# wg-perception/PartsBasedDetector

Measured on AMD Instinct MI355X. Metric: detect() frames/sec, 640x480, 26-part person model, higher is better.
Workload: dtype f32

## Files before the change

partsbaseddetector_amd/csrc/k_conv.hip:

```cpp
#include <algorithm>
#include <vector>
#include <cstring>
#include "pbd_internal.hpp"
#include <type_traits>
#include "k_conv_mfma16.hpp"

#ifdef PBD_PROBES
bool conv_variants_debug_read(unsigned long long* out);
void conv_debug_read(unsigned long long* out) {
  if (!conv_variants_debug_read(out)) hipMemcpyFromSymbol(out, HIP_SYMBOL(pbd_conv_dbg), sizeof(unsigned long long) * 8);
}
#else
void conv_debug_read(unsigned long long* out) { for (int i = 0; i < 8; ++i) out[i] = 0; }
#endif

#define CSTR 33
#define NFG 8

template <int KH, int KW>
__device__ __forceinline__ void stage_feature_tile(float* __restrict__ ft, const float* __restrict__ F, int y0, int x0,
                                                   int H, int W, int tid) {
  constexpr int TW = CT + KW - 1, TH = CT + KH - 1, N = TH * TW * 8, NB = (N + 255) / 256;
  float4 r[NB];
#pragma unroll
  for (int j = 0; j < NB; ++j) {
    const int i = min(tid + j * 256, N - 1);
    const int cell = i >> 3, q = i & 7;
    const int ty = cell / TW, tx = cell - ty * TW;
    const int y = min(max(y0 + ty - KH / 2, 0), H - 1), x = min(max(x0 + tx - KW / 2, 0), W - 1);
    r[j] = *(const float4*)(F + ((size_t)y * W + x) * PBD_FLEN + q * 4);
  }
#pragma unroll
  for (int j = 0; j < NB; ++j) {
    const int i = tid + j * 256;
    if (i < N) {
      const int cell = i >> 3, q = i & 7;
      const int ty = cell / TW, tx = cell - ty * TW;
      const int y = y0 + ty - KH / 2, x = x0 + tx - KW / 2;
      float4 v = r[j];
      if (!(y >= 0 && y < H && x >= 0 && x < W)) v = make_float4(0.f, 0.f, 0.f, q == 7 ? 1.f : 0.f);
      float* d = ft + cell * CSTR + q * 4;
      d[0] = v.x; d[1] = v.y; d[2] = v.z; d[3] = v.w;
    }
  }
}

template <int KH, int KW>
__global__ __launch_bounds__(256) void k_conv_exact(const ConvTile* __restrict__ tiles,
                                                    const LevelDev* __restrict__ levels,
                                                    const float* __restrict__ feat, const float* __restrict__ wT,
                                                    float* __restrict__ resp, int nf, int nfpad, int groups_per_wg) {
  extern __shared__ __attribute__((aligned(16))) char smem[];
  typedef float T;
  T* ft = (T*)smem;
  const ConvTile t = tiles[blockIdx.x];
  const LevelDev lv = levels[t.level];
  const int H = lv.ch, W = lv.cw;
  const int TW = CT + KW - 1;
  const int tid = threadIdx.x;
  const T* F = feat + lv.cell_off * PBD_FLEN;
  stage_feature_tile<KH, KW>(ft, F, t.y0, t.x0, H, W, tid);
  __syncthreads();
  const int ly = tid >> 4, lx = tid & 15;
  const int oy = t.y0 + ly, ox = t.x0 + lx;
  const bool valid = (oy < H && ox < W);
  const T* fbase = ft + (ly * TW + lx) * CSTR;
  T* R = resp + lv.cell_off * nf;
  const int g0 = blockIdx.y * groups_per_wg;
  for (int g = g0; g < g0 + groups_per_wg; ++g) {
    const int n0 = g * NFG;
    if (n0 >= nf) break;
    T tot[NFG];
#pragma unroll
    for (int n = 0; n < NFG; ++n) tot[n] = (T)0;
    for (int c = 0; c < PBD_FLEN; ++c) {
      T acc[NFG];
#pragma unroll
      for (int n = 0; n < NFG; ++n) acc[n] = (T)0;
#pragma unroll
      for (int i = 0; i < KH; ++i) {
#pragma unroll
        for (int j = 0; j < KW; ++j) {
          const T f = fbase[(i * TW + j) * CSTR + c];
          const T* w = wT + ((size_t)(i * KW + j) * PBD_FLEN + c) * nfpad + n0;
#pragma unroll
          for (int n = 0; n < NFG; ++n) acc[n] += w[n] * f;
        }
      }
#pragma unroll
      for (int n = 0; n < NFG; ++n) tot[n] += acc[n];
    }
    if (valid) {
#pragma unroll
      for (int n = 0; n < NFG; ++n)
        if (n0 + n < nf) R[(size_t)(n0 + n) * H * W + (size_t)oy * W + ox] = tot[n];
    }
  }
}

#define CHALF 16
#define CSTRH 17
template <int KH, int KW, int GPW>
__global__ __launch_bounds__(256) void k_conv_exact_f64(const ConvTile* __restrict__ tiles,
                                                        const LevelDev* __restrict__ levels,
                                                        const double* __restrict__ feat, const double* __restrict__ wT,
                                                        double* __restrict__ resp, int nf, int nfpad) {
  extern __shared__ __attribute__((aligned(16))) char smem[];
  double* ft = (double*)smem;
  const ConvTile t = tiles[blockIdx.x];
  const LevelDev lv = levels[t.level];
  const int H = lv.ch, W = lv.cw;
  constexpr int TW = CT + KW - 1;
  const int tid = threadIdx.x;
  const double* F = feat + lv.cell_off * PBD_FLEN;
  const int ly = tid >> 4, lx = tid & 15;
  const int oy = t.y0 + ly, ox = t.x0 + lx;
  const bool valid = (oy < H && ox < W);
  const double* fbase = ft + (ly * TW + lx) * CSTRH;
  double* R = resp + lv.cell_off * nf;
  const int g0 = blockIdx.y * GPW;
  double tot[GPW][NFG];
#pragma unroll
  for (int g = 0; g < GPW; ++g)
#pragma unroll
    for (int n = 0; n < NFG; ++n) tot[g][n] = 0.0;
  for (int half = 0; half < PBD_FLEN / CHALF; ++half) {
    if (half) __syncthreads();
    stage_tile<double, CHALF, CSTRH, 7>(ft, F, t.y0, t.x0, H, W, KH, KW, half * CHALF, half == PBD_FLEN / CHALF - 1, tid);
    __syncthreads();
#pragma unroll
    for (int g = 0; g < GPW; ++g) {
      const int n0 = (g0 + g) * NFG;
      if (n0 >= nf) break;
      for (int cc = 0; cc < CHALF; ++cc) {
        const int c = half * CHALF + cc;
        double acc[NFG];
#pragma unroll
        for (int n = 0; n < NFG; ++n) acc[n] = 0.0;
#pragma unroll
        for (int i = 0; i < KH; ++i) {
#pragma unroll
          for (int j = 0; j < KW; ++j) {
            const double f = fbase[(i * TW + j) * CSTRH + cc];
            const double* w = wT + ((size_t)(i * KW + j) * PBD_FLEN + c) * nfpad + n0;
#pragma unroll
            for (int n = 0; n < NFG; ++n) acc[n] += w[n] * f;
          }
        }
#pragma unroll
        for (int n = 0; n < NFG; ++n) tot[g][n] += acc[n];
      }
    }
  }
  if (valid) {
#pragma unroll
    for (int g = 0; g < GPW; ++g) {
      const int n0 = (g0 + g) * NFG;
#pragma unroll
      for (int n = 0; n < NFG; ++n)
        if (n0 + n < nf) R[(size_t)(n0 + n) * H * W + (size_t)oy * W + ox] = tot[g][n];
    }
  }
}

template <typename T, bool MIX = false>
__global__ __launch_bounds__(256) void k_conv_exact_generic(const ConvTile* __restrict__ tiles,
                                                            const LevelDev* __restrict__ levels,
                                                            const T* __restrict__ feat,
                                                            const T* __restrict__ wT, T* __restrict__ resp,
                                                            int nf, int nfpad, int KH, int KW) {
  extern __shared__ __attribute__((aligned(16))) char smem[];
  T* ft = (T*)smem;
  const ConvTile t = tiles[blockIdx.x];
  const LevelDev lv = levels[t.level];
  const int H = lv.ch, W = lv.cw;
  const int TW = CT + KW - 1, TH = CT + KH - 1;
  const int tid = threadIdx.x;
  const T* F = feat + lv.cell_off * PBD_FLEN;
  for (int i = tid; i < TH * TW * PBD_FLEN; i += 256) {
    const int cell = i >> 5, c = i & 31;
    const int ty = cell / TW, tx = cell - ty * TW;
    const int y = t.y0 + ty - KH / 2, x = t.x0 + tx - KW / 2;
    const bool inside = (y >= 0 && y < H && x >= 0 && x < W);
    const T v = F[((size_t)min(max(y, 0), H - 1) * W + min(max(x, 0), W - 1)) * PBD_FLEN + c];
    ft[cell * CSTR + c] = inside ? v : (T)(c == PBD_FLEN - 1 ? 1 : 0);
  }
  __syncthreads();
  const int ly = tid >> 4, lx = tid & 15;
  const int oy = t.y0 + ly, ox = t.x0 + lx;
  const bool valid = (oy < H && ox < W);
  const T* fbase = ft + (ly * TW + lx) * CSTR;
  T* R = resp + lv.cell_off * nf;
  int nfw = nf;
  if constexpr (MIX) { R += (size_t)(t.pad & 0xFFFF) * H * W; nfw = t.pad >> 16; }
  for (int n = blockIdx.y; n < nfw; n += gridDim.y) {
    T tot = (T)0;
    for (int c = 0; c < PBD_FLEN; ++c) {
      T acc = (T)0;
      for (int i = 0; i < KH; ++i)
        for (int j = 0; j < KW; ++j)
          acc += wT[((size_t)(i * KW + j) * PBD_FLEN + c) * nfpad + n] * fbase[(i * TW + j) * CSTR + c];
      tot += acc;
    }
    if (valid) R[(size_t)n * H * W + (size_t)oy * W + ox] = tot;
  }
}

template <typename T>
static void launch_conv_exact_t(const ConvTile* tiles, int ntiles, const LevelDev* levels, const T* feat,
                                const T* wT, T* resp, int nf, int nfpad, int kh, int kw, hipStream_t s, int nf_stride) {
  const size_t lds = sizeof(T) * (CT + kh - 1) * (CT + kw - 1) * CSTR;
  if (nf_stride > 0) {
    static LdsOptIn optinm;
    optinm.ensure((const void*)k_conv_exact_generic<T, true>, lds);
    dim3 grid(ntiles, nf < 16 ? nf : 16);
    hipLaunchKernelGGL((k_conv_exact_generic<T, true>), grid, dim3(256), lds, s, tiles, levels, feat, wT, resp, nf_stride, nfpad, kh, kw);
    return;
  }
  if (kh == 5 && kw == 5) {
    const int groups = (nf + NFG - 1) / NFG;
    constexpr int GPW = 4;
    dim3 grid(ntiles, (groups + GPW - 1) / GPW);
    static LdsOptIn optin;
    if constexpr (sizeof(T) == 8) {
      const size_t ldsh = sizeof(double) * (CT + 4) * (CT + 4) * CSTRH;
      optin.ensure((const void*)k_conv_exact_f64<5, 5, GPW>, ldsh);
      hipLaunchKernelGGL((k_conv_exact_f64<5, 5, GPW>), grid, dim3(256), ldsh, s, tiles, levels, feat, wT, resp, nf, nfpad);
    } else {
      optin.ensure((const void*)k_conv_exact<5, 5>, lds);
      hipLaunchKernelGGL((k_conv_exact<5, 5>), grid, dim3(256), lds, s, tiles, levels, feat, wT, resp, nf, nfpad, GPW);
    }
  } else {
    static LdsOptIn opting;
    opting.ensure((const void*)k_conv_exact_generic<T>, lds);
    dim3 grid(ntiles, nf < 16 ? nf : 16);
    hipLaunchKernelGGL(k_conv_exact_generic<T>, grid, dim3(256), lds, s, tiles, levels, feat, wT, resp, nf, nfpad, kh, kw);
  }
}

void launch_conv_exact(const ConvTile* tiles, int ntiles, const LevelDev* levels, const void* feat, const void* wT,
                       void* resp, int ts, int nf, int nfpad, int kh, int kw, hipStream_t s, int nf_stride) {
  if (ntiles <= 0) return;
  if (ts == 8) launch_conv_exact_t<double>(tiles, ntiles, levels, (const double*)feat, (const double*)wT, (double*)resp, nf, nfpad, kh, kw, s, nf_stride);
  else launch_conv_exact_t<float>(tiles, ntiles, levels, (const float*)feat, (const float*)wT, (float*)resp, nf, nfpad, kh, kw, s, nf_stride);
}

void launch_conv_mfma_f64(const ConvTile* tiles, int ntiles, const LevelDev* levels, const double* feat,
                          const double* w4u, double* resp, int nf, int nfpad, int kh, int kw, hipStream_t s, int nf_stride) {
  if (ntiles <= 0) return;
  if (nf_stride > 0)
    launch_conv_mfma16_t<double, 4, 2, 1, true, 0, 0, true>(tiles, ntiles, levels, feat, w4u, resp, nf, nfpad, s, kh, kw, nf_stride);
  else if (kh != 5 || kw != 5)
    launch_conv_mfma16_t<double, 4, 2, 1, true, 0, 0>(tiles, ntiles, levels, feat, w4u, resp, nf, nfpad, s, kh, kw);
  else
    launch_conv_mfma16_t<double, 4, 2, 1, true>(tiles, ntiles, levels, feat, w4u, resp, nf, nfpad, s);
}

void launch_conv_mfma16_f32(const ConvTile* tiles, int ntiles, const LevelDev* levels, const float* feat,
                            const float* w4u, float* resp, int nf, int nfpad, int kh, int kw, hipStream_t s, int nf_stride) {
  if (ntiles <= 0) return;
  if (nf_stride > 0)
    launch_conv_mfma16_t<float, 2, 3, 2, true, 0, 0, true>(tiles, ntiles, levels, feat, w4u, resp, nf, nfpad, s, kh, kw, nf_stride);
  else if (kh != 5 || kw != 5)
    launch_conv_mfma16_t<float, 2, 3, 2, true, 0, 0>(tiles, ntiles, levels, feat, w4u, resp, nf, nfpad, s, kh, kw);
  else
    launch_conv_mfma16_t<float, 2, 3, 2, true>(tiles, ntiles, levels, feat, w4u, resp, nf, nfpad, s);
}
```

Baseline: 2440.

## Rework f32 5x5 conv inner loop with packed float2 FMAs and prefetching

The f32 5x5 exact conv kernel now computes 16 filters per group using packed float2 vector math instead of 8 scalar filters. Weights for the next tap are loaded one step ahead through constant-address-space pointers, and feature values for the next channel are prefetched from LDS. Scheduling barriers pin the loads between FMA groups. The aim is to raise FMA throughput via packed ops and hide weight/LDS load latency. In exchange it uses more registers, which may lower occupancy, and the grid is rebalanced to 2 groups per workgroup.

New measurement: 2445, median of 2. Within noise of the previous version (+0.2%).

```diff
diff --git a/partsbaseddetector_amd/csrc/k_conv.hip b/partsbaseddetector_amd/csrc/k_conv.hip
--- a/partsbaseddetector_amd/csrc/k_conv.hip
+++ b/partsbaseddetector_amd/csrc/k_conv.hip
@@ -16,6 +16,9 @@
 
 #define CSTR 33
 #define NFG 8
+#define NFGP 16
+typedef float float2v __attribute__((ext_vector_type(2)));
+typedef const __attribute__((address_space(4))) float2v* wpair_ptr;
 
 template <int KH, int KW>
 __device__ __forceinline__ void stage_feature_tile(float* __restrict__ ft, const float* __restrict__ F, int y0, int x0,
@@ -66,34 +69,59 @@
   const bool valid = (oy < H && ox < W);
   const T* fbase = ft + (ly * TW + lx) * CSTR;
   T* R = resp + lv.cell_off * nf;
+  const size_t wtap = (size_t)PBD_FLEN * nfpad;
   const int g0 = blockIdx.y * groups_per_wg;
   for (int g = g0; g < g0 + groups_per_wg; ++g) {
-    const int n0 = g * NFG;
+    const int n0 = g * NFGP;
     if (n0 >= nf) break;
-    T tot[NFG];
-#pragma unroll
-    for (int n = 0; n < NFG; ++n) tot[n] = (T)0;
+    float2v tot[NFGP / 2];
+#pragma unroll
+    for (int p = 0; p < NFGP / 2; ++p) tot[p] = float2v{0.f, 0.f};
+    const float* w0 = wT + n0;
+    float2v wn[NFGP / 2];
+#pragma unroll
+    for (int p = 0; p < NFGP / 2; ++p) wn[p] = ((wpair_ptr)w0)[p];
+    T fn[KH * KW];
+#pragma unroll
+    for (int k = 0; k < KH * KW; ++k) fn[k] = fbase[((k / KW) * TW + k % KW) * CSTR];
     for (int c = 0; c < PBD_FLEN; ++c) {
-      T acc[NFG];
-#pragma unroll
-      for (int n = 0; n < NFG; ++n) acc[n] = (T)0;
-#pragma unroll
-      for (int i = 0; i < KH; ++i) {
-#pragma unroll
-        for (int j = 0; j < KW; ++j) {
-          const T f = fbase[(i * TW + j) * CSTR + c];
-          const T* w = wT + ((size_t)(i * KW + j) * PBD_FLEN + c) * nfpad + n0;
-#pragma unroll
-          for (int n = 0; n < NFG; ++n) acc[n] += w[n] * f;
-        }
+      T f[KH * KW];
+#pragma unroll
+      for (int k = 0; k < KH * KW; ++k) f[k] = fn[k];
+      const int cn = min(c + 1, PBD_FLEN - 1);
+#pragma unroll
+      for (int k = 0; k < KH * KW; ++k) fn[k] = fbase[((k / KW) * TW + k % KW) * CSTR + cn];
+      const float* wc = w0 + (size_t)c * nfpad;
+      float2v acc[NFGP / 2];
+#pragma unroll
+      for (int p = 0; p < NFGP / 2; ++p) acc[p] = float2v{0.f, 0.f};
+#pragma unroll
+      for (int k = 0; k < KH * KW; ++k) {
+        float2v w[NFGP / 2];
+#pragma unroll
+        for (int p = 0; p < NFGP / 2; ++p) w[p] = wn[p];
+        const float2v f2 = float2v{f[k], f[k]};
+        __builtin_amdgcn_sched_barrier(0);
+        const float2v prod0 = w[0] * f2;
+        __builtin_amdgcn_sched_barrier(0);
+        const float* wnext = k + 1 < KH * KW ? wc + (size_t)(k + 1) * wtap : wc + nfpad;
+#pragma unroll
+        for (int p = 0; p < NFGP / 2; ++p) wn[p] = ((wpair_ptr)wnext)[p];
+        __builtin_amdgcn_sched_barrier(0);
+        acc[0] += prod0;
+#pragma unroll
+        for (int p = 1; p < NFGP / 2; ++p) acc[p] += w[p] * f2;
+        __builtin_amdgcn_sched_barrier(0);
       }
 #pragma unroll
-      for (int n = 0; n < NFG; ++n) tot[n] += acc[n];
+      for (int p = 0; p < NFGP / 2; ++p) tot[p] += acc[p];
     }
     if (valid) {
 #pragma unroll
-      for (int n = 0; n < NFG; ++n)
-        if (n0 + n < nf) R[(size_t)(n0 + n) * H * W + (size_t)oy * W + ox] = tot[n];
+      for (int p = 0; p < NFGP / 2; ++p) {
+        if (n0 + 2 * p < nf) R[(size_t)(n0 + 2 * p) * H * W + (size_t)oy * W + ox] = tot[p].x;
+        if (n0 + 2 * p + 1 < nf) R[(size_t)(n0 + 2 * p + 1) * H * W + (size_t)oy * W + ox] = tot[p].y;
+      }
     }
   }
 }
@@ -218,8 +246,8 @@
     return;
   }
   if (kh == 5 && kw == 5) {
-    const int groups = (nf + NFG - 1) / NFG;
-    constexpr int GPW = 4;
+    constexpr int GPW = sizeof(T) == 8 ? 4 : 2, PER = sizeof(T) == 8 ? NFG : NFGP;
+    const int groups = (nf + PER - 1) / PER;
     dim3 grid(ntiles, (groups + GPW - 1) / GPW);
     static LdsOptIn optin;
     if constexpr (sizeof(T) == 8) {
```
